# AlanLiangC/PDM-SSD

Measured on AMD Instinct MI355X. Metric: frames/sec (16384-pt clouds, bs=32), higher is better.
Workload: dtype f32; 1 GPU; configs[2]: full PDM-SSD forward (PointNet2MSG backbone + PDM neck + hybrid head: BEV heat-map head + point box head with decoded boxes), bs=32/GPU x 16384 pts, uniform KITTI-range clouds, fp32 inference, inputs resident in HBM, 4 distinct batches in rotation; launch=hipGraph, parallelism=dp1, global_batch=32

## Files before the change

include/pdmssd_hip.h:

```cpp
#ifndef PDMSSD_HIP_H
#define PDMSSD_HIP_H

#include <stddef.h>

#ifdef __cplusplus
extern "C" {
#endif

#define PDM_ABI_VERSION 1

#define PDM_E_BADARG (-1)
#define PDM_E_TOOLARGE (-2)

int pdm_abi_version(void);
const char *pdm_last_error(void);


int pdm_ball_query(void *stream, int b, int n, int m, float radius, int nsample,
                   const float *new_xyz, const float *xyz, int *idx);

int pdm_group_points(void *stream, int b, int c, int n, int npoints, int nsample,
                     const float *points, const int *idx, float *out);

int pdm_group_points_grad(void *stream, int b, int c, int n, int npoints, int nsample,
// ... 106 lines not shown
                        size_t workspace_bytes);
size_t pdm_point_head_loss_workspace_bytes(long long n_total);

int pdm_heatmap_targets(void *stream, int B, int M, int C, int H, int W, const float *gt_boxes, float x0, float y0, float vx,
                        float vy, float stride, double min_overlap, int min_radius, int max_radius, float *heatmap);
size_t pdm_heatmap_focal_loss_workspace_bytes(long long n);
int pdm_heatmap_focal_loss(void *stream, int B, int C, int H, int W, const void *logits, int logits_bf16, long long sb, long long sc,
                           long long sh, long long sw, const float *heatmap, float weight, float *dlogits, float *out,
                           void *workspace, size_t workspace_bytes);

int pdm_rows_mlp_x3(void *stream, int rows, int cin, const float *in_pm, int nlayers, const int *dims, const void *wstream,
                    size_t wstream_bytes, const float *bias, int relu_last, float *out_pm, int out_stride, int cout);
size_t pdm_rows_mlp_x3_stream_bytes(int nlayers, const int *dims);
int pdm_tune_rows_x3_wg_per_cu(int n);

int pdm_sa_mlp_fused_pre(void *stream, int b, int n, int m, int nsample, const float *xyz,
                         const float *new_xyz, const float *z_pm, int z_stride, int z_coff, const int *idx,
                         int nlayers, const int *dims, const float *wpack, const float *bias, float *out_pm,
                         int out_stride, int out_coff, int cout);
int pdm_fp_mlp_fused_pre(void *stream, int b, int n, int m, int c_skip, const float *z_pm, int z_stride,
                         const float *skip_pm, const int *idx, const float *weight, int nlayers,
                         const int *dims, const float *wpack, const float *bias, float *out_pm,
                         int out_stride, int cout);

size_t pdm_sa_pack_workspace_bytes(int b, int m);
size_t pdm_sa_pack_rows(int b, int m, int nsample);
int pdm_sa_pack(void *stream, int b, int n, int m, int nsample, const int *idx, void *workspace,
                size_t workspace_bytes, int *pack, int *meta);
int pdm_sa_pack_pair(void *stream, int b, int n, int m, const int *nsample, const int *const *idx, void *const *workspace,
                     size_t workspace_bytes, int *const *pack, int *const *meta);
int pdm_sa_mlp_packed(void *stream, int b, int n, int m, int cin, int nsample, const float *xyz,
                      const float *new_xyz, const float *feat_pm, const float *z_pm, int z_stride, int z_coff,
                      const int *pack, const int *meta, int nlayers, const int *dims, const float *wpack,
                      const float *bias, float *out_pm, int out_stride, int out_coff, int cout);

int pdm_sa_mlp_packed_pair(void *stream, int b, int n, int m, int cin, const int *nsample, const float *xyz,
                           const float *new_xyz, const float *feat_pm, const float *z_pm, int z_stride, const int *z_coff,
                           const int *const *pack, const int *const *meta, const int *nlayers, const int *const *dims,
                           const float *const *wpack, const float *const *bias, float *out_pm, int out_stride,
                           const int *out_coff, const int *cout);
int pdm_tune_sa_pair(int on);

int pdm_stack_ball_query(void *stream, int B, int M, float radius, int nsample, const float *new_xyz,
                         const int *new_xyz_batch_cnt, const float *xyz, const int *xyz_batch_cnt, int *idx);
int pdm_stack_group_points(void *stream, int B, int M, int C, int nsample, const float *features,
                           const int *features_batch_cnt, const int *idx, const int *idx_batch_cnt, float *out);
// ... 140 lines not shown
                        void *xmin, unsigned char *imax, unsigned char *imin);
int pdm_tg_dy_stats_parts(long long rows, int N);
int pdm_tg_gemm_nt_dy_bs(void *stream, long long R, int K, int N, const void *dZ, long long lddz, const void *Yp, long long ldyp,
                         const void *W, long long ldw, void *dX, long long lddx, void *dYout, long long lddy, const float *coef,
                         const float *grads, const void *Bx, long long ldbx, const float *bcoef, float *bstats);
size_t pdm_tg_wgrad_ws_bytes(long long R, int K, int N);
int pdm_tg_wgrad(void *stream, long long R, int K, int N, const void *dY, long long ldy, const void *X, long long ldx, float *dW,
                 int accumulate, void *workspace, size_t workspace_bytes, const float *x_bn_coef);
size_t pdm_tg_colsum_ws_floats(long long R, int N);
int pdm_tg_colsum(void *stream, long long R, int N, const void *Y, long long ld, float *out, float *scratch);
int pdm_tg_pack_weight(void *stream, int N, int K, const float *W, void *Wb, int ldb, void *Wt, int ldt);
int pdm_tg_pack_weight_pair(void *stream, int N, int K, const float *W, void *Wb, void *Wt, int rows_to, int cols_to);
int pdm_tg_pack_weight_many(void *stream, int njobs, const void *jobs, long long total_blocks);


int pdm_tune_fps_variant(int v);
int pdm_tune_fused_waves(int w);
int pdm_tune_fused_tiles(int t);
int pdm_tune_fused_groups(int n);
int pdm_tune_fused_wg_per_cu(int n);
int pdm_tune_fused_lds_cap(int bytes);
int pdm_tune_fused_reg(int on);
int pdm_tune_fused_gemm(int on);
int pdm_tune_fused_chain(int on);
int pdm_tune_fused_swz(int on);
int pdm_tune_bq_quad(int form);
int pdm_tune_bq_dense_ppc(int hundredths);
int pdm_tune_grid_split(int min_n);
int pdm_tune_bq_small_waves(int w);
int pdm_tune_bq_cpw(int centres);
int pdm_tune_bq_heavy(int candidates);
int pdm_tune_group_lds_floor(int bytes);
int pdm_tune_group_rows(int packed);
int pdm_tune_rows_chain_wg_per_cu(int n);
int pdm_tune_fp_head_tiles(int n);
int pdm_tune_rows_chain_dw_wg_per_cu(int n);
int pdm_tune_rows_chain_xcd(int on);
int pdm_tune_fp_chain_pad_lds(int bytes);

int pdm_copy_many(void *stream, int count, void *const *dst, const void *const *src, const size_t *bytes);
int pdm_copy_many_dyn(void *stream, int count, void *const *dst, const void *const *src, const size_t *bytes,
                      const int *const *dyn_count, const unsigned *dyn_unit);


int pdm_scatter_bev(void *stream, int B, int P, int C, int degree, const float *xyz,
                    const float *feat, const float *sh, const float *inv2s2, float ox, float oy,
// ... 37 lines not shown
```

pdm_ssd_amd/_native.py:

```python
import ctypes
import os

import torch

_HERE = os.path.dirname(os.path.abspath(__file__))
LIB_PATH = os.path.join(_HERE, "libpdmssd_hip.so")
ABI_VERSION = 1

_lib = None

_vp, _i, _f = ctypes.c_void_p, ctypes.c_int, ctypes.c_float

_SIGNATURES = {
    "pdm_ball_query": [_i, _i, _i, _f, _i, _vp, _vp, _vp],
    "pdm_ball_query_grid": [_i, _i, _i, _f, _i, _vp, _vp, _vp, _vp, ctypes.c_size_t],
    "pdm_grid_build": [_i, _i, _f, _vp, _vp, ctypes.c_size_t],
    "pdm_ball_query_grid_prebuilt": [_i, _i, _i, _f, _i, _vp, _vp, _vp, ctypes.c_size_t],
    "pdm_three_nn_grid_prebuilt": [_i, _i, _i, _vp, _vp, _vp, _vp, ctypes.c_size_t],
    "pdm_three_nn_grid": [_i, _i, _i, _vp, _vp, _vp, _vp, _vp, ctypes.c_size_t],
    "pdm_group_points": [_i, _i, _i, _i, _i, _vp, _vp, _vp],
    "pdm_group_points_grad": [_i, _i, _i, _i, _i, _vp, _vp, _vp],
    "pdm_group_points_grad_ws": [_i, _i, _i, _i, _i, _vp, _vp, _vp, _vp, ctypes.c_size_t],
    "pdm_gather_points": [_i, _i, _i, _i, _vp, _vp, _vp],
    "pdm_gather_points_grad": [_i, _i, _i, _i, _vp, _vp, _vp],
# ... 55 lines not shown
    "pdm_bn_relu_backward_stats": [_i, _i, ctypes.c_longlong, _i, ctypes.c_longlong, _vp, _vp, _vp, _vp, _vp, _i],
    "pdm_bn_relu_backward_apply": [_i, _i, ctypes.c_longlong, _i, ctypes.c_longlong, _vp, _vp, _vp, _vp, _vp, _i],
    "pdm_stack_voxel_query": [_i, _i, _i, _i, _i, _f, _i, _i, _i, _vp, _vp, _vp, _vp, _vp],
    "pdm_stack_local_neighbor_count": [_vp, _vp, _vp, _vp, _vp, _vp, _f, _i, _i, _i, _i],
    "pdm_stack_local_neighbor_fill": [_vp, _vp, _vp, _vp, _vp, _vp, ctypes.c_longlong, _f, _i, _i, _i, _i],
    "pdm_stack_query_local_neighbor_idxs": [_vp, _vp, _vp, _vp, _vp, _vp, _vp, _i, _f, _i, _i, _i, _i],
    "pdm_stack_three_nn_by_local_idxs": [_vp, _vp, _vp, _vp, _vp, _vp, ctypes.c_longlong, _i, _i],
    "pdm_stack_vector_pool_count": [_vp] * 7 + [_i, _i, _i, _f, _i, _i, _i, _i, _i],
    "pdm_stack_vector_pool": [_vp] * 10 + [_i, _i, _i, _f] + [_i] * 9,
    "pdm_stack_vector_pool_grad": [_vp, _vp, _vp, _vp, _i, _i, _i, _i, _i, _i],
    "pdm_three_nn_weights": [ctypes.c_longlong, _vp, _vp, _vp],
    "pdm_rows_mlp_fused": [_i, _i, _vp, _i, _vp, _vp, _vp, _i, _vp, _i, _i],
    "pdm_point_head_loss": [ctypes.c_longlong, _i, _i, _i, _i, _i, _vp, ctypes.c_longlong, _vp, ctypes.c_longlong, _vp, ctypes.c_longlong,
                            _vp, _vp, _vp, _vp, _vp, _f, _f, _f, _f, _f, _vp, _vp, _vp, _vp, _vp, ctypes.c_size_t],
    "pdm_heatmap_targets": [_i, _i, _i, _i, _i, _vp, _f, _f, _f, _f, _f, ctypes.c_double, _i, _i, _vp],
    "pdm_heatmap_focal_loss": [_i, _i, _i, _i, _vp, _i, ctypes.c_longlong, ctypes.c_longlong, ctypes.c_longlong, ctypes.c_longlong, _vp, _f, _vp, _vp,
                               _vp, ctypes.c_size_t],
    "pdm_rows_mlp_x3": [_i, _i, _vp, _i, _vp, _vp, ctypes.c_size_t, _vp, _i, _vp, _i, _i],
    "pdm_rows_mlp_fused_pair": [_i, _i, _vp, _i, _vp, _vp, _vp, _vp, _vp, _i, _vp, _i, _i, _vp, _i, _i],
    "pdm_fp_head_fused": [_i, _i, _i, _i, _vp, _i, _vp, _vp, _vp, _vp, _vp, _vp, _vp, _i, _i, _vp, _vp, _vp, _vp, _vp, _i, _vp, _i, _i,
                          _vp, _i, _i],
    "pdm_sa_mlp_fused_pre": [_i] * 4 + [_vp, _vp, _vp, _i, _i, _vp, _i, _vp, _vp, _vp, _vp, _i, _i, _i],
    "pdm_fp_mlp_fused_pre": [_i] * 4 + [_vp, _i, _vp, _vp, _vp, _i, _vp, _vp, _vp, _vp, _i, _i],
    "pdm_sa_pack": [_i, _i, _i, _i, _vp, _vp, ctypes.c_size_t, _vp, _vp],
    "pdm_sa_pack_pair": [_i, _i, _i, _vp, _vp, _vp, ctypes.c_size_t, _vp, _vp],
    "pdm_sa_mlp_packed_pair": [_i, _i, _i, _i, _vp, _vp, _vp, _vp, _vp, _i, _vp, _vp, _vp, _vp, _vp, _vp, _vp, _vp, _i, _vp, _vp],
    "pdm_sa_mlp_packed": [_i] * 5 + [_vp, _vp, _vp, _vp, _i, _i, _vp, _vp, _i, _vp, _vp, _vp, _vp, _i, _i, _i],
    "pdm_interp_concat_rows": [_i, _i, _i, _i, _i, _i, _vp, _i, _vp, _i, _vp, _vp, _vp],
    "pdm_interp_concat_rows_grad": [_i, _i, _i, _i, _i, _vp, _vp, _vp, _vp, _vp, ctypes.c_size_t],
    "pdm_interp_concat_rows_grad_out": [_i, _i, _i, _i, _i, _vp, _vp, _vp, _vp, _i, _vp, ctypes.c_size_t],
    "pdm_tg_gemm_nt": [ctypes.c_longlong, _i, _i, _vp, ctypes.c_longlong, _vp, ctypes.c_longlong, _vp, ctypes.c_longlong, _vp, _vp, _vp],
    "pdm_tg_gemm_nt_dy": [ctypes.c_longlong, _i, _i, _vp, ctypes.c_longlong, _vp, ctypes.c_longlong, _vp, ctypes.c_longlong, _vp, ctypes.c_longlong,
                          _vp, ctypes.c_longlong, _vp, _vp],
    "pdm_tg_gemm_nt_bs": [ctypes.c_longlong, _i, _i, _vp, ctypes.c_longlong, _vp, ctypes.c_longlong, _vp, ctypes.c_longlong, _vp,
                          ctypes.c_longlong, _vp, _vp],
    "pdm_tg_gemm_nt_dy_bs": [ctypes.c_longlong, _i, _i, _vp, ctypes.c_longlong, _vp, ctypes.c_longlong, _vp, ctypes.c_longlong, _vp,
                             ctypes.c_longlong, _vp, ctypes.c_longlong, _vp, _vp, _vp, ctypes.c_longlong, _vp, _vp],
    "pdm_bn_finalize_bwd_stats": [ctypes.c_longlong, _i, _vp, _vp, _vp, _i],
    "pdm_tg_gemm_nt_pool": [ctypes.c_longlong, _i, _i, _vp, ctypes.c_longlong, _vp, ctypes.c_longlong, _vp, ctypes.c_longlong, _vp, _vp, _vp,
                            _i, _vp, _vp, _vp, _vp],
    "pdm_bn_relu_pool_forward_kept": [_i, ctypes.c_longlong, _i, _i, _vp, _vp, _vp, _vp, _vp, _f, _f, _vp, _vp, _vp, _vp, _i, _i],
    "pdm_tg_wgrad": [ctypes.c_longlong, _i, _i, _vp, ctypes.c_longlong, _vp, ctypes.c_longlong, _vp, _i, _vp, ctypes.c_size_t, _vp],
    "pdm_bn_forward_coef": [_i, ctypes.c_longlong, _i, _vp, _vp, _vp, _f, _f, _vp, _vp, _vp, _vp],
    "pdm_bn_finalize_stats": [ctypes.c_longlong, _i, _vp, _vp, _f, _f, _vp, _vp, _vp, _vp, _i],
    "pdm_tg_colsum": [ctypes.c_longlong, _i, _vp, ctypes.c_longlong, _vp, _vp],
    "pdm_tg_pack_weight": [_i, _i, _vp, _vp, _i, _vp, _i],
    "pdm_tg_pack_weight_pair": [_i, _i, _vp, _vp, _vp, _i, _i],
    "pdm_tg_pack_weight_many": [_i, _vp, ctypes.c_longlong],
    "pdm_tune_fps_variant": None,
    "pdm_tune_fused_waves": None,
    "pdm_tune_fused_tiles": None,
    "pdm_tune_fused_groups": None,
    "pdm_tune_fused_wg_per_cu": None,
    "pdm_tune_fused_lds_cap": None,
    "pdm_tune_fused_reg": None,
    "pdm_tune_bq_quad": None,
    "pdm_tune_bq_heavy": None,
    "pdm_tune_bq_cpw": None,
    "pdm_tune_copy_variant": None,
    "pdm_tune_group_nt": None,
    "pdm_tune_group_lds_floor": None,
    "pdm_tune_copy_max_wg": None,
    "pdm_tune_bq_small_waves": None,
    "pdm_tune_bq_dense_ppc": None,
    "pdm_tune_grid_split": None,
    "pdm_tune_group_rows": None,
    "pdm_tune_fused_gemm": None,
    "pdm_tune_fused_chain": None,
    "pdm_tune_fused_pair": None,
    "pdm_tune_sa_pair": None,
    "pdm_tune_rows_x3_wg_per_cu": None,
    "pdm_tune_fp_chain_pad_lds": None,
    "pdm_tune_fp_chain_nt": None,
    "pdm_tune_fp_chain_mask": None,
    "pdm_tune_rows_chain_wg_per_cu": None,
    "pdm_tune_rows_chain_dw_wg_per_cu": None,
    "pdm_tune_fp_head_tiles": None,
    "pdm_tune_rows_chain_xcd": None,
    "pdm_tune_fused_swz": None,
    "pdm_scatter_bev": [_i, _i, _i, _i, _vp, _vp, _vp, _vp] + [_f] * 9 + [_i] * 7 + [_vp, _vp],
    "pdm_gather_bev": [_i, _i, _i, _i, _vp, _vp, _vp, _vp] + [_f] * 9 + [_i] * 6 + [_i, _f, _vp, _vp, _vp, ctypes.c_size_t],
    "pdm_bev_normalize_grad": [_i, _i, _i, _i, _i, _f, _vp, _vp, _vp, _vp, _vp],
    "pdm_bev_normalize": [_i, _i, _i, _i, _i, _i, _f, _vp, _vp],
    "pdm_scatter_bev_grad": [_i, _i, _i, _i, _vp, _vp, _vp, _vp] + [_f] * 9 + [_i] * 7 + [_vp] * 5,
    "pdm_scatter_bev_grad_normalized": [_i, _i, _i, _i, _vp, _vp, _vp, _vp] + [_f] * 9 + [_i] * 7 + [_vp, _vp, _f] + [_vp] * 4,
}
EXPORTS = ["pdm_abi_version", "pdm_last_error", "pdm_ball_query_grid_workspace_bytes",
           "pdm_three_nn_grid_workspace_bytes", "pdm_furthest_point_sampling_ws_bytes",
           "pdm_fps_max_coresident_workgroups",
           "pdm_gather_bev_workspace_bytes", "pdm_nms_workspace_bytes", "pdm_post_process_workspace_bytes", "pdm_augment_workspace_bytes", "pdm_sa_pack_workspace_bytes",
           "pdm_sa_pack_rows", "pdm_rows_mlp_x3_stream_bytes", "pdm_point_head_loss_workspace_bytes", "pdm_heatmap_focal_loss_workspace_bytes", "pdm_three_interpolate_grad_ws_bytes",
           "pdm_group_points_grad_ws_bytes", "pdm_group_concat_cl_grad_ws_bytes", "pdm_bn_parts", "pdm_bn_pool_parts",
           "pdm_tg_stats_parts", "pdm_tg_dy_stats_parts", "pdm_tg_wgrad_ws_bytes", "pdm_tg_colsum_ws_floats"] + list(_SIGNATURES)


class NativeLibraryError(RuntimeError):
    pass


def lib():
    global _lib
    if _lib is None:
        if not os.path.exists(LIB_PATH):
            raise NativeLibraryError(
                f"{LIB_PATH} not found: build it with `make -C pdm_ssd_amd/csrc` "
                "(or `python -c 'import __graft_entry__ as g; g.build()'`). "
                "pdm_ssd_amd has no CPU or PyTorch fallback for its operators.")
        l = ctypes.CDLL(LIB_PATH)
        l.pdm_abi_version.restype = _i
        l.pdm_last_error.restype = ctypes.c_char_p
        l.pdm_ball_query_grid_workspace_bytes.restype = ctypes.c_size_t
        l.pdm_ball_query_grid_workspace_bytes.argtypes = [_i, _i]
        l.pdm_furthest_point_sampling_ws_bytes.restype = ctypes.c_size_t
        l.pdm_furthest_point_sampling_ws_bytes.argtypes = [_i, _i]
        l.pdm_fps_max_coresident_workgroups.restype = _i
        l.pdm_fps_max_coresident_workgroups.argtypes = []
# ... 5 lines not shown
        l.pdm_sa_pack_workspace_bytes.restype = ctypes.c_size_t
        l.pdm_sa_pack_workspace_bytes.argtypes = [_i, _i]
        l.pdm_group_concat_cl_grad_ws_bytes.restype = ctypes.c_size_t
        l.pdm_group_concat_cl_grad_ws_bytes.argtypes = [_i, _i, _i, _i]
        l.pdm_group_points_grad_ws_bytes.restype = ctypes.c_size_t
        l.pdm_group_points_grad_ws_bytes.argtypes = [_i, _i, _i, _i]
        l.pdm_three_interpolate_grad_ws_bytes.restype = ctypes.c_size_t
        l.pdm_three_interpolate_grad_ws_bytes.argtypes = [_i, _i, _i]
        l.pdm_point_head_loss_workspace_bytes.restype = ctypes.c_size_t
        l.pdm_point_head_loss_workspace_bytes.argtypes = [ctypes.c_longlong]
        l.pdm_heatmap_focal_loss_workspace_bytes.restype = ctypes.c_size_t
        l.pdm_heatmap_focal_loss_workspace_bytes.argtypes = [ctypes.c_longlong]
        l.pdm_rows_mlp_x3_stream_bytes.restype = ctypes.c_size_t
        l.pdm_rows_mlp_x3_stream_bytes.argtypes = [_i, _vp]
        l.pdm_sa_pack_rows.restype = ctypes.c_size_t
        l.pdm_sa_pack_rows.argtypes = [_i, _i, _i]
        l.pdm_nms_workspace_bytes.argtypes = [_i]
        l.pdm_post_process_workspace_bytes.restype = ctypes.c_size_t
        l.pdm_post_process_workspace_bytes.argtypes = [_i, _i, _i]
        l.pdm_augment_workspace_bytes.restype = ctypes.c_size_t
        l.pdm_augment_workspace_bytes.argtypes = [_i, _i]
        l.pdm_bn_pool_parts.restype = _i
        l.pdm_bn_pool_parts.argtypes = [_i, ctypes.c_longlong, _i]
        l.pdm_tg_colsum_ws_floats.restype = ctypes.c_size_t
        l.pdm_tg_colsum_ws_floats.argtypes = [ctypes.c_longlong, _i]
        l.pdm_tg_stats_parts.restype = _i
        l.pdm_tg_stats_parts.argtypes = [ctypes.c_longlong, _i]
        l.pdm_tg_dy_stats_parts.restype = _i
        l.pdm_tg_dy_stats_parts.argtypes = [ctypes.c_longlong, _i]
        l.pdm_tg_wgrad_ws_bytes.restype = ctypes.c_size_t
        l.pdm_tg_wgrad_ws_bytes.argtypes = [ctypes.c_longlong, _i, _i]
        l.pdm_bn_parts.restype = _i
        l.pdm_bn_parts.argtypes = [_i, ctypes.c_longlong, _i, ctypes.c_longlong]
        if l.pdm_abi_version() != ABI_VERSION:
            raise NativeLibraryError(
                f"libpdmssd_hip.so ABI {l.pdm_abi_version()} != expected {ABI_VERSION}; rebuild it")
        for name, args in _SIGNATURES.items():
            fn = getattr(l, name)
            fn.restype = _i
            fn.argtypes = [_i] if args is None else [_vp] + args
        _lib = l
    return _lib


def call(name, stream, *args):
    l = lib()
# ... 68 lines not shown
```

pdm_ssd_amd/csrc/fused_mlp.hip:

```cpp
#include "common.h"

#include <mutex>
#include <set>

namespace pdm {

typedef float f4 __attribute__((ext_vector_type(4)));

constexpr int FM_MAXL = 4;

struct MlpDesc {
    int nlayers;
    int K[FM_MAXL + 1];
    int woff[FM_MAXL];
    int boff[FM_MAXL];
    int stage_in;
    int pool_floats;
    int relu_last;
    int lds_p, lds_q;
    int swz;
};

__device__ __forceinline__ int lds_col(int blk, int g, int pos, int swz) {
    const int q = 4 * blk + g;
// ... 1011 lines not shown
            } else {
#pragma unroll
                for (int t = 0; t < NT; ++t) v[t] = seg_max_nonneg4(v[t], L[t]);
            }
            const int c0 = 16 * mb + 4 * g;
#pragma unroll
            for (int t = 0; t < NT; ++t) {
                if (!orow[t]) continue;
                if (c0 + 4 <= a.cout) {
                    *reinterpret_cast<f4 *>(orow[t] + c0) = v[t];
                } else {
                    if (c0 < a.cout) orow[t][c0] = v[t].x;
                    if (c0 + 1 < a.cout) orow[t][c0 + 1] = v[t].y;
                    if (c0 + 2 < a.cout) orow[t][c0 + 2] = v[t].z;
                }
            }
        }
    }
#undef PDM_CHAIN
}

int rows_gemm_launch(void *stream, int rows, int cin, const float *in_pm, int k0, int c1, const float *wpack,
                     const float *bias, int relu_last, float *out_pm, int out_stride, int cout);
int rows_chain_launch(void *stream, int rows, int cin, const float *in_pm, int nlayers, const int *dims, const float *wpack,
                      const float *bias, int relu_last, float *out_pm, int out_stride, int cout, int *launched);
int rows_chain_pair_launch(void *stream, int rows, int cin, const float *in_pm, int nlayers, const int *dims, const float *wpack_a,
                           const float *bias_a, const float *wpack_b, const float *bias_b, int relu_last, float *out_a, int out_stride_a,
                           int cout_a, float *out_b, int out_stride_b, int cout_b, int *launched);
static int g_fused_chain = 1;
static int g_fused_pair = 1;
int fp_chain_launch(void *stream, int b, int n, int m, int c_skip, const float *z_pm, int z_stride, const float *skip_pm,
                    const int *idx, const float *weight, const int *dims, const float *wpack, const float *bias, float *out_pm,
                    int out_stride, int cout, int *launched);
int fp_pre_gemm_launch(void *stream, int b, int n, int m, int c_skip, const float *z_pm, int z_stride,
                       const float *skip_pm, const int *idx, const float *weight, int k1, int c2,
                       const float *wpack, const float *bias, float *out_pm, int out_stride, int cout);
static int g_fused_swz = 1;
static int g_fused_gemm = 1;
static int g_fused_reg = 1;
static int g_fused_waves = 0;
static int g_fused_tiles = 0;
static int g_fused_groups = 0;
static int g_fused_lds_cap = 152 * 1024;
static int g_fused_wg_per_cu = 32;

static int fill_desc(const char *who, MlpDesc &d, int nlayers, const int *dims, int k0_real_max, int pool_floats,
// ... 323 lines not shown

extern "C" int pdm_fp_mlp_fused_pre(void *stream, int b, int n, int m, int c_skip, const float *z_pm,
                                    int z_stride, const float *skip_pm, const int *idx, const float *weight,
                                    int nlayers, const int *dims, const float *wpack, const float *bias,
                                    float *out_pm, int out_stride, int cout) {
    return fp_fused_launch(stream, 1, 1, b, n, m, 0, c_skip, nullptr, z_pm, z_stride, skip_pm, idx, weight, nlayers, dims,
                           wpack, bias, out_pm, out_stride, cout);
}

extern "C" int pdm_rows_mlp_fused(void *stream, int rows, int cin, const float *in_pm, int nlayers,
                                  const int *dims, const float *wpack, const float *bias, int relu_last,
                                  float *out_pm, int out_stride, int cout) {
    PDM_REQUIRE(rows >= 0 && cin >= 1, PDM_E_BADARG, "rows_mlp_fused: rows=%d cin=%d", rows, cin);
    if (g_fused_chain && dims && in_pm && wpack && bias && out_pm && cout > 0 && nlayers >= 1 && nlayers <= 3 && cout <= dims[nlayers] &&
        cout <= out_stride && out_stride % 4 == 0 &&
        ((reinterpret_cast<uintptr_t>(out_pm) | reinterpret_cast<uintptr_t>(wpack) | reinterpret_cast<uintptr_t>(bias) |
          reinterpret_cast<uintptr_t>(in_pm)) & 15) == 0) {
        int launched = 0;
        const int rc = rows_chain_launch(stream, rows, cin, in_pm, nlayers, dims, wpack, bias, relu_last, out_pm, out_stride, cout,
                                         &launched);
        if (rc || launched) return rc;
    }
    if (g_fused_gemm && nlayers == 1 && dims && dims[0] % 16 == 0 && dims[1] % 16 == 0 && dims[0] >= cin && dims[0] >= 32 &&
        dims[1] >= 64 && (long long)((rows + 127) / 128) * ((dims[1] + 127) / 128) >= 256 && in_pm && wpack && bias && out_pm && cout > 0 && cout <= dims[1] && cout <= out_stride &&
        out_stride % 4 == 0 && ((reinterpret_cast<uintptr_t>(out_pm) | reinterpret_cast<uintptr_t>(wpack) |
                                 reinterpret_cast<uintptr_t>(bias)) & 15) == 0)
        return rows_gemm_launch(stream, rows, cin, in_pm, dims[0], dims[1], wpack, bias, relu_last, out_pm, out_stride, cout);
    return fp_fused_launch(stream, 2, relu_last, 1, rows, 1, 0, cin, nullptr, nullptr, 0, in_pm, nullptr, nullptr, nlayers,
                           dims, wpack, bias, out_pm, out_stride, cout);
}

extern "C" int pdm_rows_mlp_fused_pair(void *stream, int rows, int cin, const float *in_pm, int nlayers, const int *dims,
                                       const float *wpack_a, const float *bias_a, const float *wpack_b, const float *bias_b,
                                       int relu_last, float *out_a, int out_stride_a, int cout_a, float *out_b, int out_stride_b,
                                       int cout_b) {
    PDM_REQUIRE(rows >= 0 && cin >= 1, PDM_E_BADARG, "rows_mlp_fused_pair: rows=%d cin=%d", rows, cin);
    if (g_fused_chain && g_fused_pair && dims && in_pm && wpack_a && bias_a && wpack_b && bias_b && out_a && out_b && out_a != out_b &&
        nlayers == 3 && cout_a > 0 && cout_b > 0 && cout_a <= dims[nlayers] && cout_b <= dims[nlayers] && cout_a <= out_stride_a &&
        cout_b <= out_stride_b && out_stride_a % 4 == 0 && out_stride_b % 4 == 0 &&
        ((reinterpret_cast<uintptr_t>(out_a) | reinterpret_cast<uintptr_t>(out_b) | reinterpret_cast<uintptr_t>(wpack_a) |
          reinterpret_cast<uintptr_t>(wpack_b) | reinterpret_cast<uintptr_t>(bias_a) | reinterpret_cast<uintptr_t>(bias_b) |
          reinterpret_cast<uintptr_t>(in_pm)) & 15) == 0) {
        int launched = 0;
        const int rc = rows_chain_pair_launch(stream, rows, cin, in_pm, nlayers, dims, wpack_a, bias_a, wpack_b, bias_b, relu_last, out_a,
                                              out_stride_a, cout_a, out_b, out_stride_b, cout_b, &launched);
        if (rc || launched) return rc;
    }
    if (int rc = pdm_rows_mlp_fused(stream, rows, cin, in_pm, nlayers, dims, wpack_a, bias_a, relu_last, out_a, out_stride_a, cout_a)) return rc;
    return pdm_rows_mlp_fused(stream, rows, cin, in_pm, nlayers, dims, wpack_b, bias_b, relu_last, out_b, out_stride_b, cout_b);
}
// ... 1 lines not shown
```

pdm_ssd_amd/csrc/rows_gemm.hip:

```cpp
#include "common.h"

namespace pdm {

typedef float gf4 __attribute__((ext_vector_type(4)));

constexpr int RG_ROWS = 128;
constexpr int RG_BLKS = 8;
constexpr int RG_HS = 24;

struct RowsGemmArgs {
    int rows, cin, in_stride;
    int nkb, nmb;
    int cout, out_stride;
    const float *in;
    const float *wpack;
    const float *bias;
    float *out;
    float floor;
    int n, m, z_stride, c_skip;
    const float *z;
    const float *skip;
    const int *idx;
    const float *weight;
    const float *w1;
    const float *b1;
};

template <bool FP_PRE>
__global__ __launch_bounds__(512) void rows_gemm_kernel(RowsGemmArgs a) {
    __shared__ __attribute__((aligned(16))) float s_w[2][RG_BLKS * 64 * 4];
    __shared__ __attribute__((aligned(16))) float s_h[2][RG_ROWS * RG_HS];
    const int tid = threadIdx.x, lane = tid & 63;
    const int wave = __builtin_amdgcn_readfirstlane(tid >> 6);
    const int pos = lane & 15, g = lane >> 4;
    const int wp = wave >> 2, wc = wave & 3;
    int tile = blockIdx.x;
    if constexpr (FP_PRE) {
        const int tpc = a.n / RG_ROWS, nb = a.rows / a.n;
        if (gridDim.y == 1 && tpc * RG_ROWS == a.n && (nb & 7) == 0) {
            const int xcd = tile & 7, slot = tile >> 3;
            tile = ((slot / tpc) * 8 + xcd) * tpc + slot % tpc;
        }
    }
    const long long r0 = (long long)tile * RG_ROWS;
    const int mb0 = blockIdx.y * RG_BLKS;

    const int hrow = tid >> 2, part = tid & 3;
    const bool w_live = mb0 + wave < a.nmb;
    const gf4 *wsrc = reinterpret_cast<const gf4 *>(a.wpack) + ((size_t)(mb0 + wave) * a.nkb) * 64 + lane;
    const bool h_live = r0 + hrow < a.rows;
    const float *hsrc = a.in + (size_t)(r0 + hrow) * a.in_stride + 4 * part;
    const bool vec = (a.in_stride & 3) == 0 && (reinterpret_cast<uintptr_t>(a.in) & 15) == 0;

    auto load_w = [&](int kb) {
        gf4 v = {0.f, 0.f, 0.f, 0.f};
        if (w_live) v = wsrc[(size_t)kb * 64];
        return v;
    };
    const float *zb = nullptr;
    int o0 = 0, o1 = 0, o2 = 0;
    float iw0 = 0.f, iw1 = 0.f, iw2 = 0.f, sk[4] = {0.f, 0.f, 0.f, 0.f};
    if constexpr (FP_PRE) {
        if (h_live) {
            const long long row = r0 + hrow;
            const int b = (int)(row / a.n);
            zb = a.z + (size_t)b * a.m * a.z_stride + 4 * part;
            o0 = a.idx[row * 3] * a.z_stride; o1 = a.idx[row * 3 + 1] * a.z_stride; o2 = a.idx[row * 3 + 2] * a.z_stride;
            iw0 = a.weight[row * 3]; iw1 = a.weight[row * 3 + 1]; iw2 = a.weight[row * 3 + 2];
            for (int s_ = 0; s_ < a.c_skip; ++s_) sk[s_] = a.skip[row * a.c_skip + s_];
        }
    }
    struct Raw { gf4 za, zc, zd; };
    auto load_raw = [&](int kb) {
// ... 16 lines not shown
#pragma unroll
        for (int j = 0; j < 4; ++j) {
            h[j] += __fmaf_rn(iw2, zz[2][j], __fmaf_rn(iw1, zz[1][j], __fmul_rn(iw0, zz[0][j])));
            const float *wr = a.w1 + ((size_t)(c >> 4) * 64 + ((c & 15) + j)) * 4;
            for (int s_ = 0; s_ < a.c_skip; ++s_) h[j] = fmaf(wr[s_], sk[s_], h[j]);
            h[j] = fmaxf(h[j], 0.0f);
        }
        return gf4{h[0], h[1], h[2], h[3]};
    };
    auto load_h = [&](int kb) {
        gf4 v = {0.f, 0.f, 0.f, 0.f};
        if (!h_live) return v;
        const int c = 16 * kb + 4 * part;
        if (vec && c + 4 <= a.cin) return *reinterpret_cast<const gf4 *>(hsrc + 16 * kb);
        const float *p = hsrc + 16 * kb;
        if (c < a.cin) v.x = p[0];
        if (c + 1 < a.cin) v.y = p[1];
        if (c + 2 < a.cin) v.z = p[2];
        if (c + 3 < a.cin) v.w = p[3];
        return v;
    };
    auto stage = [&](int buf, gf4 w, gf4 h) {
        reinterpret_cast<gf4 *>(s_w[buf])[tid] = w;
        *reinterpret_cast<gf4 *>(&s_h[buf][hrow * RG_HS + 4 * part]) = h;
    };

    gf4 acc[2][4];
#pragma unroll
    for (int i = 0; i < 2; ++i) {
        gf4 bi = {0.f, 0.f, 0.f, 0.f};
        if (mb0 + 2 * wc + i < a.nmb) bi = *reinterpret_cast<const gf4 *>(a.bias + 16 * (mb0 + 2 * wc + i) + 4 * g);
#pragma unroll
        for (int t = 0; t < 4; ++t) acc[i][t] = bi;
    }

    gf4 gw = load_w(0), gh = {0.f, 0.f, 0.f, 0.f};
    Raw gr;
    if constexpr (FP_PRE) { gr = load_raw(0); gh = finish(gr, 0); } else gh = load_h(0);
    stage(0, gw, gh);
    __syncthreads();
    if (a.nkb > 1) {
        gw = load_w(1);
        if constexpr (FP_PRE) gr = load_raw(1); else gh = load_h(1);
    }
    for (int kb = 0; kb < a.nkb; ++kb) {
        const int cur = kb & 1;
        gf4 fa[2], fb[4];
#pragma unroll
        for (int i = 0; i < 2; ++i) fa[i] = reinterpret_cast<const gf4 *>(s_w[cur])[(2 * wc + i) * 64 + lane];
#pragma unroll
        for (int t = 0; t < 4; ++t) fb[t] = *reinterpret_cast<const gf4 *>(&s_h[cur][((4 * wp + t) * 16 + pos) * RG_HS + 4 * g]);
        if (kb + 1 < a.nkb) {
            if constexpr (FP_PRE) gh = finish(gr, kb + 1);
            stage(cur ^ 1, gw, gh);
        }
        if (kb + 2 < a.nkb) {
            gw = load_w(kb + 2);
            if constexpr (FP_PRE) gr = load_raw(kb + 2); else gh = load_h(kb + 2);
        }
#define PDM_RG_MFMA(C)                                                                                         \
    _Pragma("unroll") for (int i = 0; i < 2; ++i) _Pragma("unroll") for (int t = 0; t < 4; ++t)                 \
        acc[i][t] = __builtin_amdgcn_mfma_f32_16x16x4f32(fa[i].C, fb[t].C, acc[i][t], 0, 0, 0);
        PDM_RG_MFMA(x) PDM_RG_MFMA(y) PDM_RG_MFMA(z) PDM_RG_MFMA(w)
#undef PDM_RG_MFMA
        __syncthreads();
    }

#pragma unroll
    for (int t = 0; t < 4; ++t) {
        const long long row = r0 + (4 * wp + t) * 16 + pos;
        if (row >= a.rows) continue;
        float *orow = a.out + (size_t)row * a.out_stride;
#pragma unroll
        for (int i = 0; i < 2; ++i) {
            const int c0 = 16 * (mb0 + 2 * wc + i) + 4 * g;
            gf4 v = acc[i][t];
            v.x = __builtin_amdgcn_fmed3f(v.x, a.floor, __builtin_inff()); v.y = __builtin_amdgcn_fmed3f(v.y, a.floor, __builtin_inff());
            v.z = __builtin_amdgcn_fmed3f(v.z, a.floor, __builtin_inff()); v.w = __builtin_amdgcn_fmed3f(v.w, a.floor, __builtin_inff());
            if (c0 + 4 <= a.cout) {
                *reinterpret_cast<gf4 *>(orow + c0) = v;
            } else {
                if (c0 < a.cout) orow[c0] = v.x;
                if (c0 + 1 < a.cout) orow[c0 + 1] = v.y;
                if (c0 + 2 < a.cout) orow[c0 + 2] = v.z;
            }
        }
    }
}

int rows_gemm_launch(void *stream, int rows, int cin, const float *in_pm, int k0, int c1, const float *wpack,
                     const float *bias, int relu_last, float *out_pm, int out_stride, int cout) {
    RowsGemmArgs a;
    a.rows = rows; a.cin = cin; a.in_stride = cin;
    a.nkb = k0 >> 4; a.nmb = c1 >> 4;
    a.cout = cout; a.out_stride = out_stride;
    a.in = in_pm; a.wpack = wpack; a.bias = bias; a.out = out_pm;
    a.floor = relu_last ? 0.0f : -__builtin_inff();
    a.n = a.m = a.z_stride = a.c_skip = 0;
    a.z = a.skip = a.weight = a.w1 = a.b1 = nullptr; a.idx = nullptr;
    const dim3 grid((unsigned)((rows + RG_ROWS - 1) / RG_ROWS), (unsigned)((a.nmb + RG_BLKS - 1) / RG_BLKS));
    hipLaunchKernelGGL(rows_gemm_kernel<false>, grid, dim3(512), 0, as_stream(stream), a);
    return check_launch("rows_mlp_fused(gemm)");
}

int fp_pre_gemm_launch(void *stream, int b, int n, int m, int c_skip, const float *z_pm, int z_stride,
                       const float *skip_pm, const int *idx, const float *weight, int k1, int c2,
                       const float *wpack, const float *bias, float *out_pm, int out_stride, int cout) {
    RowsGemmArgs a;
    a.rows = b * n; a.cin = k1; a.in_stride = 0;
    a.nkb = k1 >> 4; a.nmb = c2 >> 4;
    a.cout = cout; a.out_stride = out_stride;
    a.in = nullptr; a.wpack = wpack + 16 * k1; a.bias = bias + k1; a.out = out_pm;
    a.floor = 0.0f;
    a.n = n; a.m = m; a.z_stride = z_stride; a.c_skip = c_skip;
    a.z = z_pm; a.skip = skip_pm; a.idx = idx; a.weight = weight; a.w1 = wpack; a.b1 = bias;
    const dim3 grid((unsigned)((a.rows + RG_ROWS - 1) / RG_ROWS), (unsigned)((a.nmb + RG_BLKS - 1) / RG_BLKS));
    hipLaunchKernelGGL(rows_gemm_kernel<true>, grid, dim3(512), 0, as_stream(stream), a);
    return check_launch("fp_mlp_fused_pre(gemm)");
}

}
```

pdm_ssd_amd/fused.py:

```python
import ctypes

import numpy as np
import torch
import torch.nn as nn

from . import _native

FLOP_COUNTER = None


def _count(name, positions, pk):
    if FLOP_COUNTER is not None:
        FLOP_COUNTER[name] = FLOP_COUNTER.get(name, 0.0) + float(positions) * pk.flops_per_position


def _pad16(c):
    return (c + 15) // 16 * 16


def fold_conv_bn(conv, bn):
    w = conv.weight.detach().double().reshape(conv.out_channels, conv.in_channels).cpu()
    if conv.bias is not None:
        cb = conv.bias.detach().double().cpu()
    else:
# ... 373 lines not shown
def sa_level_forward_packed(pks, xyz, new_xyz, feat_pm, z, z_coffs, packeds, nss, out_pm, out_coffs):
    B, N, _ = xyz.shape
    M = new_xyz.shape[1]
    cin = 0 if (feat_pm is None or z is not None) else feat_pm.shape[2]
    assert len(pks) == 2 and all(pk.cin == cin + 3 for pk in pks)
    if FLOP_COUNTER is not None:
        for pk, (pack, meta) in zip(pks, packeds):
            _count("pdm_sa_mlp_packed_pair", int(meta[6].item()), pk)
    I2, P2 = ctypes.c_int * 2, ctypes.c_void_p * 2
    keep = [I2(*nss), I2(*z_coffs), P2(*[p.data_ptr() for p, _ in packeds]), P2(*[m.data_ptr() for _, m in packeds]),
            I2(*[pk.nlayers for pk in pks]), P2(*[pk.dims_ptr.value for pk in pks]), P2(*[pk.wpack.data_ptr() for pk in pks]),
            P2(*[pk.bias.data_ptr() for pk in pks]), I2(*out_coffs), I2(*[pk.cout for pk in pks])]
    c = [ctypes.cast(k, ctypes.c_void_p) for k in keep]
    _native.call("pdm_sa_mlp_packed_pair", _stream(xyz), B, N, M, cin, c[0], xyz.data_ptr(), new_xyz.data_ptr(),
                 0 if cin == 0 else feat_pm.data_ptr(), 0 if z is None else z.data_ptr(), 0 if z is None else z.shape[2], c[1], c[2], c[3],
                 c[4], c[5], c[6], c[7], out_pm.data_ptr(), out_pm.shape[2], c[8], c[9])


def fp_forward_pre(pk, z, skip_pm, idx, weight, out_pm):
    B, m, _ = z.shape
    n = idx.shape[1]
    cs = 0 if skip_pm is None else skip_pm.shape[2]
    assert pk.cin == cs
    _count("pdm_fp_mlp_fused_pre", B * n, pk)
    _native.call("pdm_fp_mlp_fused_pre", _stream(z), B, n, m, cs, z.data_ptr(), z.shape[2],
                 0 if skip_pm is None else skip_pm.data_ptr(), idx.data_ptr(), weight.data_ptr(), pk.nlayers,
                 pk.dims_ptr, pk.wpack.data_ptr(), pk.bias.data_ptr(), out_pm.data_ptr(), out_pm.shape[2], pk.cout)
```

Before: 7272 frames/s.

## Add small-row-tile GEMM forms and split FP pre-MLP into interp-fused two-GEMM path

Templates the rows GEMM kernel on row-tile size (128/64/32) so under-filled launches with large K and N use smaller tiles and produce more workgroups. Adds a workspace-based FP pre path that runs the first layer as a GEMM on skip features, adds the three-NN interpolated z in the epilogue, and runs the second layer as a separate GEMM. This replaces the single fused pre kernel when grids would be small. It costs an intermediate workspace round trip through HBM and a torch allocation per call.

```diff
diff --git a/include/pdmssd_hip.h b/include/pdmssd_hip.h
--- a/include/pdmssd_hip.h
+++ b/include/pdmssd_hip.h
@@ -152,6 +152,11 @@
                          const float *skip_pm, const int *idx, const float *weight, int nlayers,
                          const int *dims, const float *wpack, const float *bias, float *out_pm,
                          int out_stride, int cout);
+size_t pdm_fp_mlp_pre_ws_floats(int b, int n, int c_skip, int nlayers, const int *dims);
+int pdm_fp_mlp_fused_pre_ws(void *stream, int b, int n, int m, int c_skip, const float *z_pm, int z_stride,
+                            const float *skip_pm, const int *idx, const float *weight, int nlayers,
+                            const int *dims, const float *wpack, const float *bias, float *out_pm,
+                            int out_stride, int cout, float *ws, size_t ws_floats);
 
 size_t pdm_sa_pack_workspace_bytes(int b, int m);
 size_t pdm_sa_pack_rows(int b, int m, int nsample);
@@ -338,6 +343,7 @@
 int pdm_tune_fused_lds_cap(int bytes);
 int pdm_tune_fused_reg(int on);
 int pdm_tune_fused_gemm(int on);
+int pdm_tune_rows_gemm_forms(int on);
 int pdm_tune_fused_chain(int on);
 int pdm_tune_fused_swz(int on);
 int pdm_tune_bq_quad(int form);
diff --git a/pdm_ssd_amd/_native.py b/pdm_ssd_amd/_native.py
--- a/pdm_ssd_amd/_native.py
+++ b/pdm_ssd_amd/_native.py
@@ -101,6 +101,7 @@
                           _vp, _i, _i],
     "pdm_sa_mlp_fused_pre": [_i] * 4 + [_vp, _vp, _vp, _i, _i, _vp, _i, _vp, _vp, _vp, _vp, _i, _i, _i],
     "pdm_fp_mlp_fused_pre": [_i] * 4 + [_vp, _i, _vp, _vp, _vp, _i, _vp, _vp, _vp, _vp, _i, _i],
+    "pdm_fp_mlp_fused_pre_ws": [_i] * 4 + [_vp, _i, _vp, _vp, _vp, _i, _vp, _vp, _vp, _vp, _i, _i, _vp, ctypes.c_size_t],
     "pdm_sa_pack": [_i, _i, _i, _i, _vp, _vp, ctypes.c_size_t, _vp, _vp],
     "pdm_sa_pack_pair": [_i, _i, _i, _vp, _vp, _vp, ctypes.c_size_t, _vp, _vp],
     "pdm_sa_mlp_packed_pair": [_i, _i, _i, _i, _vp, _vp, _vp, _vp, _vp, _i, _vp, _vp, _vp, _vp, _vp, _vp, _vp, _vp, _i, _vp, _vp],
@@ -133,6 +134,7 @@
     "pdm_tune_fused_wg_per_cu": None,
     "pdm_tune_fused_lds_cap": None,
     "pdm_tune_fused_reg": None,
+    "pdm_tune_rows_gemm_forms": None,
     "pdm_tune_bq_quad": None,
     "pdm_tune_bq_heavy": None,
     "pdm_tune_bq_cpw": None,
@@ -170,7 +172,7 @@
            "pdm_gather_bev_workspace_bytes", "pdm_nms_workspace_bytes", "pdm_post_process_workspace_bytes", "pdm_augment_workspace_bytes", "pdm_sa_pack_workspace_bytes",
            "pdm_sa_pack_rows", "pdm_rows_mlp_x3_stream_bytes", "pdm_point_head_loss_workspace_bytes", "pdm_heatmap_focal_loss_workspace_bytes", "pdm_three_interpolate_grad_ws_bytes",
            "pdm_group_points_grad_ws_bytes", "pdm_group_concat_cl_grad_ws_bytes", "pdm_bn_parts", "pdm_bn_pool_parts",
-           "pdm_tg_stats_parts", "pdm_tg_dy_stats_parts", "pdm_tg_wgrad_ws_bytes", "pdm_tg_colsum_ws_floats"] + list(_SIGNATURES)
+           "pdm_tg_stats_parts", "pdm_tg_dy_stats_parts", "pdm_tg_wgrad_ws_bytes", "pdm_tg_colsum_ws_floats", "pdm_fp_mlp_pre_ws_floats"] + list(_SIGNATURES)
 
 
 class NativeLibraryError(RuntimeError):
@@ -222,6 +224,8 @@
         l.pdm_augment_workspace_bytes.argtypes = [_i, _i]
         l.pdm_bn_pool_parts.restype = _i
         l.pdm_bn_pool_parts.argtypes = [_i, ctypes.c_longlong, _i]
+        l.pdm_fp_mlp_pre_ws_floats.restype = ctypes.c_size_t
+        l.pdm_fp_mlp_pre_ws_floats.argtypes = [_i, _i, _i, _i, _vp]
         l.pdm_tg_colsum_ws_floats.restype = ctypes.c_size_t
         l.pdm_tg_colsum_ws_floats.argtypes = [ctypes.c_longlong, _i]
         l.pdm_tg_stats_parts.restype = _i
diff --git a/pdm_ssd_amd/csrc/fused_mlp.hip b/pdm_ssd_amd/csrc/fused_mlp.hip
--- a/pdm_ssd_amd/csrc/fused_mlp.hip
+++ b/pdm_ssd_amd/csrc/fused_mlp.hip
@@ -1057,6 +1057,9 @@
 
 int rows_gemm_launch(void *stream, int rows, int cin, const float *in_pm, int k0, int c1, const float *wpack,
                      const float *bias, int relu_last, float *out_pm, int out_stride, int cout);
+bool rows_gemm_tiles_apply(int rows, int k0, int c1);
+int rows_gemm_tiles_launch(void *stream, int rows, int cin, const float *in_pm, int k0, int c1, const float *wpack,
+                           const float *bias, int relu_last, float *out_pm, int out_stride, int cout);
 int rows_chain_launch(void *stream, int rows, int cin, const float *in_pm, int nlayers, const int *dims, const float *wpack,
                       const float *bias, int relu_last, float *out_pm, int out_stride, int cout, int *launched);
 int rows_chain_pair_launch(void *stream, int rows, int cin, const float *in_pm, int nlayers, const int *dims, const float *wpack_a,
@@ -1426,10 +1429,15 @@
         if (rc || launched) return rc;
     }
     if (g_fused_gemm && nlayers == 1 && dims && dims[0] % 16 == 0 && dims[1] % 16 == 0 && dims[0] >= cin && dims[0] >= 32 &&
-        dims[1] >= 64 && (long long)((rows + 127) / 128) * ((dims[1] + 127) / 128) >= 256 && in_pm && wpack && bias && out_pm && cout > 0 && cout <= dims[1] && cout <= out_stride &&
+        dims[1] >= 64 && in_pm && wpack && bias && out_pm && cout > 0 && cout <= dims[1] && cout <= out_stride &&
         out_stride % 4 == 0 && ((reinterpret_cast<uintptr_t>(out_pm) | reinterpret_cast<uintptr_t>(wpack) |
-                                 reinterpret_cast<uintptr_t>(bias)) & 15) == 0)
-        return rows_gemm_launch(stream, rows, cin, in_pm, dims[0], dims[1], wpack, bias, relu_last, out_pm, out_stride, cout);
+                                 reinterpret_cast<uintptr_t>(bias)) & 15) == 0) {
+        if (rows_gemm_tiles_apply(rows, dims[0], dims[1]))
+            return rows_gemm_tiles_launch(stream, rows, cin, in_pm, dims[0], dims[1], wpack, bias, relu_last, out_pm, out_stride,
+                                          cout);
+        if ((long long)((rows + 127) / 128) * ((dims[1] + 127) / 128) >= 256)
+            return rows_gemm_launch(stream, rows, cin, in_pm, dims[0], dims[1], wpack, bias, relu_last, out_pm, out_stride, cout);
+    }
     return fp_fused_launch(stream, 2, relu_last, 1, rows, 1, 0, cin, nullptr, nullptr, 0, in_pm, nullptr, nullptr, nlayers,
                            dims, wpack, bias, out_pm, out_stride, cout);
 }
diff --git a/pdm_ssd_amd/csrc/rows_gemm.hip b/pdm_ssd_amd/csrc/rows_gemm.hip
--- a/pdm_ssd_amd/csrc/rows_gemm.hip
+++ b/pdm_ssd_amd/csrc/rows_gemm.hip
@@ -26,29 +26,34 @@
     const float *b1;
 };
 
-template <bool FP_PRE>
-__global__ __launch_bounds__(512) void rows_gemm_kernel(RowsGemmArgs a) {
+template <int ROWS, bool FP_PRE, bool INTERP = false>
+__device__ __forceinline__ void rows_gemm_body(const RowsGemmArgs &a) {
+    static_assert(ROWS == 128 || ROWS == 64 || ROWS == 32, "row tile");
+    static_assert(!FP_PRE || ROWS == 128, "the FP_PRE form stages with all 512 threads");
+    static_assert(!INTERP || (ROWS <= 64 && !FP_PRE), "INTERP keeps 24 RT registers of gathered z in flight");
+    constexpr int RT = ROWS / 32;
     __shared__ __attribute__((aligned(16))) float s_w[2][RG_BLKS * 64 * 4];
-    __shared__ __attribute__((aligned(16))) float s_h[2][RG_ROWS * RG_HS];
+    __shared__ __attribute__((aligned(16))) float s_h[2][ROWS * RG_HS];
     const int tid = threadIdx.x, lane = tid & 63;
     const int wave = __builtin_amdgcn_readfirstlane(tid >> 6);
     const int pos = lane & 15, g = lane >> 4;
     const int wp = wave >> 2, wc = wave & 3;
     int tile = blockIdx.x;
     if constexpr (FP_PRE) {
-        const int tpc = a.n / RG_ROWS, nb = a.rows / a.n;
-        if (gridDim.y == 1 && tpc * RG_ROWS == a.n && (nb & 7) == 0) {
+        const int tpc = a.n / ROWS, nb = a.rows / a.n;
+        if (gridDim.y == 1 && tpc * ROWS == a.n && (nb & 7) == 0) {
             const int xcd = tile & 7, slot = tile >> 3;
             tile = ((slot / tpc) * 8 + xcd) * tpc + slot % tpc;
         }
     }
-    const long long r0 = (long long)tile * RG_ROWS;
+    const long long r0 = (long long)tile * ROWS;
     const int mb0 = blockIdx.y * RG_BLKS;
 
     const int hrow = tid >> 2, part = tid & 3;
     const bool w_live = mb0 + wave < a.nmb;
     const gf4 *wsrc = reinterpret_cast<const gf4 *>(a.wpack) + ((size_t)(mb0 + wave) * a.nkb) * 64 + lane;
-    const bool h_live = r0 + hrow < a.rows;
+    const bool h_role = ROWS == 128 || hrow < ROWS;
+    const bool h_live = h_role && r0 + hrow < a.rows;
     const float *hsrc = a.in + (size_t)(r0 + hrow) * a.in_stride + 4 * part;
     const bool vec = (a.in_stride & 3) == 0 && (reinterpret_cast<uintptr_t>(a.in) & 15) == 0;
 
@@ -111,16 +116,42 @@
     };
     auto stage = [&](int buf, gf4 w, gf4 h) {
         reinterpret_cast<gf4 *>(s_w[buf])[tid] = w;
-        *reinterpret_cast<gf4 *>(&s_h[buf][hrow * RG_HS + 4 * part]) = h;
-    };
-
-    gf4 acc[2][4];
+        if (h_role) *reinterpret_cast<gf4 *>(&s_h[buf][hrow * RG_HS + 4 * part]) = h;
+    };
+
+    gf4 acc[2][RT];
 #pragma unroll
     for (int i = 0; i < 2; ++i) {
         gf4 bi = {0.f, 0.f, 0.f, 0.f};
         if (mb0 + 2 * wc + i < a.nmb) bi = *reinterpret_cast<const gf4 *>(a.bias + 16 * (mb0 + 2 * wc + i) + 4 * g);
 #pragma unroll
-        for (int t = 0; t < 4; ++t) acc[i][t] = bi;
+        for (int t = 0; t < RT; ++t) acc[i][t] = bi;
+    }
+
+    constexpr int ZT = INTERP ? RT : 1;
+    gf4 zp[ZT][2][3];
+    float zw[ZT][3];
+    if constexpr (INTERP) {
+#pragma unroll
+        for (int t = 0; t < RT; ++t) {
+            const long long row = r0 + (RT * wp + t) * 16 + pos;
+            const bool live = row < a.rows;
+            const long long rr = live ? row : 0;
+            const float *zb = a.z + (size_t)(rr / a.n) * a.m * a.z_stride;
+            const float *zr[3] = {zb + (size_t)a.idx[rr * 3] * a.z_stride, zb + (size_t)a.idx[rr * 3 + 1] * a.z_stride,
+                                  zb + (size_t)a.idx[rr * 3 + 2] * a.z_stride};
+#pragma unroll
+            for (int k = 0; k < 3; ++k) zw[t][k] = a.weight[rr * 3 + k];
+#pragma unroll
+            for (int i = 0; i < 2; ++i) {
+                const int mb = mb0 + 2 * wc + i;
+#pragma unroll
+                for (int k = 0; k < 3; ++k) {
+                    zp[t][i][k] = gf4{0.f, 0.f, 0.f, 0.f};
+                    if (live && mb < a.nmb) zp[t][i][k] = *reinterpret_cast<const gf4 *>(zr[k] + 16 * mb + 4 * g);
+                }
+            }
+        }
     }
 
     gf4 gw = load_w(0), gh = {0.f, 0.f, 0.f, 0.f};
@@ -134,11 +165,11 @@
     }
     for (int kb = 0; kb < a.nkb; ++kb) {
         const int cur = kb & 1;
-        gf4 fa[2], fb[4];
+        gf4 fa[2], fb[RT];
 #pragma unroll
         for (int i = 0; i < 2; ++i) fa[i] = reinterpret_cast<const gf4 *>(s_w[cur])[(2 * wc + i) * 64 + lane];
 #pragma unroll
-        for (int t = 0; t < 4; ++t) fb[t] = *reinterpret_cast<const gf4 *>(&s_h[cur][((4 * wp + t) * 16 + pos) * RG_HS + 4 * g]);
+        for (int t = 0; t < RT; ++t) fb[t] = *reinterpret_cast<const gf4 *>(&s_h[cur][((RT * wp + t) * 16 + pos) * RG_HS + 4 * g]);
         if (kb + 1 < a.nkb) {
             if constexpr (FP_PRE) gh = finish(gr, kb + 1);
             stage(cur ^ 1, gw, gh);
@@ -148,7 +179,7 @@
             if constexpr (FP_PRE) gr = load_raw(kb + 2); else gh = load_h(kb + 2);
         }
 #define PDM_RG_MFMA(C)                                                                                         \
-    _Pragma("unroll") for (int i = 0; i < 2; ++i) _Pragma("unroll") for (int t = 0; t < 4; ++t)                 \
+    _Pragma("unroll") for (int i = 0; i < 2; ++i) _Pragma("unroll") for (int t = 0; t < RT; ++t)                \
         acc[i][t] = __builtin_amdgcn_mfma_f32_16x16x4f32(fa[i].C, fb[t].C, acc[i][t], 0, 0, 0);
         PDM_RG_MFMA(x) PDM_RG_MFMA(y) PDM_RG_MFMA(z) PDM_RG_MFMA(w)
 #undef PDM_RG_MFMA
@@ -156,14 +187,23 @@
     }
 
 #pragma unroll
-    for (int t = 0; t < 4; ++t) {
-        const long long row = r0 + (4 * wp + t) * 16 + pos;
+    for (int t = 0; t < RT; ++t) {
+        const long long row = r0 + (RT * wp + t) * 16 + pos;
         if (row >= a.rows) continue;
         float *orow = a.out + (size_t)row * a.out_stride;
 #pragma unroll
         for (int i = 0; i < 2; ++i) {
             const int c0 = 16 * (mb0 + 2 * wc + i) + 4 * g;
             gf4 v = acc[i][t];
+            if constexpr (INTERP) {
+                if (mb0 + 2 * wc + i >= a.nmb) continue;
+                const gf4 p0 = zp[t][i][0], p1 = zp[t][i][1], p2 = zp[t][i][2];
+                const float w0 = zw[t][0], w1 = zw[t][1], w2 = zw[t][2];
+                v.x += __fmaf_rn(w2, p2.x, __fmaf_rn(w1, p1.x, __fmul_rn(w0, p0.x)));
+                v.y += __fmaf_rn(w2, p2.y, __fmaf_rn(w1, p1.y, __fmul_rn(w0, p0.y)));
+                v.z += __fmaf_rn(w2, p2.z, __fmaf_rn(w1, p1.z, __fmul_rn(w0, p0.z)));
+                v.w += __fmaf_rn(w2, p2.w, __fmaf_rn(w1, p1.w, __fmul_rn(w0, p0.w)));
+            }
             v.x = __builtin_amdgcn_fmed3f(v.x, a.floor, __builtin_inff()); v.y = __builtin_amdgcn_fmed3f(v.y, a.floor, __builtin_inff());
             v.z = __builtin_amdgcn_fmed3f(v.z, a.floor, __builtin_inff()); v.w = __builtin_amdgcn_fmed3f(v.w, a.floor, __builtin_inff());
             if (c0 + 4 <= a.cout) {
@@ -176,6 +216,15 @@
         }
     }
 }
+
+template <bool FP_PRE>
+__global__ __launch_bounds__(512) void rows_gemm_kernel(RowsGemmArgs a) { rows_gemm_body<RG_ROWS, FP_PRE>(a); }
+template <int ROWS>
+__global__ __launch_bounds__(512) void rows_gemm_tile_kernel(RowsGemmArgs a) { rows_gemm_body<ROWS, false>(a); }
+template <int ROWS>
+__global__ __launch_bounds__(512) void rows_gemm_interp_kernel(RowsGemmArgs a) { rows_gemm_body<ROWS, false, true>(a); }
+
+static int g_rows_gemm_tiles = 1;
 
 int rows_gemm_launch(void *stream, int rows, int cin, const float *in_pm, int k0, int c1, const float *wpack,
                      const float *bias, int relu_last, float *out_pm, int out_stride, int cout) {
@@ -191,6 +240,88 @@
     hipLaunchKernelGGL(rows_gemm_kernel<false>, grid, dim3(512), 0, as_stream(stream), a);
     return check_launch("rows_mlp_fused(gemm)");
 }
+
+static int rows_gemm_small_tile(int rows, int c1) {
+    const long long cblk = (c1 / 16 + RG_BLKS - 1) / RG_BLKS;
+    if (!g_rows_gemm_tiles || rows <= 0 || (long long)(rows + 127) / 128 * cblk >= 512) return 0;
+    return (long long)(rows + 63) / 64 * cblk >= 512 ? 64 : 32;
+}
+bool rows_gemm_tiles_apply(int rows, int k0, int c1) { return k0 >= 256 && c1 >= 256 && rows_gemm_small_tile(rows, c1) != 0; }
+int rows_gemm_tiles_launch(void *stream, int rows, int cin, const float *in_pm, int k0, int c1, const float *wpack,
+                           const float *bias, int relu_last, float *out_pm, int out_stride, int cout) {
+    RowsGemmArgs a;
+    a.rows = rows; a.cin = cin; a.in_stride = cin;
+    a.nkb = k0 >> 4; a.nmb = c1 >> 4;
+    a.cout = cout; a.out_stride = out_stride;
+    a.in = in_pm; a.wpack = wpack; a.bias = bias; a.out = out_pm;
+    a.floor = relu_last ? 0.0f : -__builtin_inff();
+    a.n = a.m = a.z_stride = a.c_skip = 0;
+    a.z = a.skip = a.weight = a.w1 = a.b1 = nullptr; a.idx = nullptr;
+    const int rt = rows_gemm_small_tile(rows, c1);
+    const dim3 grid((unsigned)((rows + rt - 1) / rt), (unsigned)((a.nmb + RG_BLKS - 1) / RG_BLKS));
+    if (rt == 64) hipLaunchKernelGGL(rows_gemm_tile_kernel<64>, grid, dim3(512), 0, as_stream(stream), a);
+    else hipLaunchKernelGGL(rows_gemm_tile_kernel<32>, grid, dim3(512), 0, as_stream(stream), a);
+    return check_launch("rows_mlp_fused(gemm tiles)");
+}
+
+static long long fp_two_gemm_ws_floats(int b, int n, int c_skip, int nlayers, const int *dims) {
+    if (!g_rows_gemm_tiles || b <= 0 || n <= 0 || nlayers != 2 || !dims || c_skip < 16) return 0;
+    for (int l = 0; l <= 2; ++l)
+        if (dims[l] <= 0 || dims[l] % 16) return 0;
+    if (dims[0] < c_skip || dims[1] < 384 || dims[2] < 256) return 0;
+    const long long rows = (long long)b * n;
+    if (rows >= (1ll << 31) || rows * dims[1] >= (1ll << 40)) return 0;
+    if ((rows + RG_ROWS - 1) / RG_ROWS * ((dims[2] / 16 + RG_BLKS - 1) / RG_BLKS) < 512) return 0;
+    return rows * dims[1];
+}
+
+}
+
+using namespace pdm;
+
+extern "C" size_t pdm_fp_mlp_pre_ws_floats(int b, int n, int c_skip, int nlayers, const int *dims) {
+    return (size_t)fp_two_gemm_ws_floats(b, n, c_skip, nlayers, dims);
+}
+
+extern "C" int pdm_fp_mlp_fused_pre(void *stream, int b, int n, int m, int c_skip, const float *z_pm, int z_stride,
+                                    const float *skip_pm, const int *idx, const float *weight, int nlayers, const int *dims,
+                                    const float *wpack, const float *bias, float *out_pm, int out_stride, int cout);
+extern "C" int pdm_fp_mlp_fused_pre_ws(void *stream, int b, int n, int m, int c_skip, const float *z_pm, int z_stride,
+                                       const float *skip_pm, const int *idx, const float *weight, int nlayers,
+                                       const int *dims, const float *wpack, const float *bias, float *out_pm,
+                                       int out_stride, int cout, float *ws, size_t ws_floats) {
+    const long long need = fp_two_gemm_ws_floats(b, n, c_skip, nlayers, dims);
+    if (need == 0 || !ws || ws_floats < (size_t)need)
+        return pdm_fp_mlp_fused_pre(stream, b, n, m, c_skip, z_pm, z_stride, skip_pm, idx, weight, nlayers, dims, wpack, bias,
+                                    out_pm, out_stride, cout);
+    PDM_REQUIRE(m >= 1 && z_pm && skip_pm && idx && weight && wpack && bias && out_pm, PDM_E_BADARG,
+                "fp_mlp_fused_pre_ws: null pointer or m=%d", m);
+    const int k1 = dims[1], c2 = dims[2];
+    PDM_REQUIRE(z_stride % 4 == 0 && z_stride >= k1 && (long long)m * z_stride < (1ll << 31), PDM_E_BADARG,
+                "fp_mlp_fused_pre_ws: z rows need %d floats, stride %d (multiple of 4)", k1, z_stride);
+    PDM_REQUIRE(cout > 0 && cout <= c2 && cout <= out_stride && out_stride % 4 == 0, PDM_E_BADARG,
+                "fp_mlp_fused_pre_ws: cout=%d stride=%d", cout, out_stride);
+    PDM_REQUIRE(((reinterpret_cast<uintptr_t>(z_pm) | reinterpret_cast<uintptr_t>(out_pm) | reinterpret_cast<uintptr_t>(ws) |
+                  reinterpret_cast<uintptr_t>(wpack) | reinterpret_cast<uintptr_t>(bias)) & 15) == 0,
+                PDM_E_BADARG, "fp_mlp_fused_pre_ws: buffers must be 16-byte aligned");
+    const int rows = b * n;
+    RowsGemmArgs a;
+    a.rows = rows; a.cin = c_skip; a.in_stride = c_skip;
+    a.nkb = dims[0] >> 4; a.nmb = k1 >> 4;
+    a.cout = k1; a.out_stride = k1;
+    a.in = skip_pm; a.wpack = wpack; a.bias = bias; a.out = ws;
+    a.floor = 0.0f;
+    a.n = n; a.m = m; a.z_stride = z_stride; a.c_skip = 0;
+    a.z = z_pm; a.idx = idx; a.weight = weight; a.skip = nullptr; a.w1 = a.b1 = nullptr;
+    const int rt = (long long)(rows + 63) / 64 * ((a.nmb + RG_BLKS - 1) / RG_BLKS) >= 512 ? 64 : 32;
+    const dim3 grid((unsigned)((rows + rt - 1) / rt), (unsigned)((a.nmb + RG_BLKS - 1) / RG_BLKS));
+    if (rt == 64) hipLaunchKernelGGL(rows_gemm_interp_kernel<64>, grid, dim3(512), 0, as_stream(stream), a);
+    else hipLaunchKernelGGL(rows_gemm_interp_kernel<32>, grid, dim3(512), 0, as_stream(stream), a);
+    if (int rc = check_launch("fp_mlp_fused_pre_ws(layer 1)")) return rc;
+    return rows_gemm_launch(stream, rows, k1, ws, k1, c2, wpack + (size_t)dims[0] * k1, bias + k1, 1, out_pm, out_stride, cout);
+}
+
+namespace pdm {
 
 int fp_pre_gemm_launch(void *stream, int b, int n, int m, int c_skip, const float *z_pm, int z_stride,
                        const float *skip_pm, const int *idx, const float *weight, int k1, int c2,
@@ -209,3 +340,5 @@
 }
 
 }
+
+extern "C" int pdm_tune_rows_gemm_forms(int on) { const int old = g_rows_gemm_tiles; g_rows_gemm_tiles = on != 0; return old; }
diff --git a/pdm_ssd_amd/fused.py b/pdm_ssd_amd/fused.py
--- a/pdm_ssd_amd/fused.py
+++ b/pdm_ssd_amd/fused.py
@@ -419,6 +419,15 @@
     n = idx.shape[1]
     cs = 0 if skip_pm is None else skip_pm.shape[2]
     assert pk.cin == cs
+    ws_floats = _native.lib().pdm_fp_mlp_pre_ws_floats(B, n, cs, pk.nlayers, pk.dims_ptr)
+    if ws_floats:
+        ws = torch.empty(ws_floats, dtype=torch.float32, device=z.device)
+        _count("pdm_fp_mlp_fused_pre_ws", B * n, pk)
+        _native.call("pdm_fp_mlp_fused_pre_ws", _stream(z), B, n, m, cs, z.data_ptr(), z.shape[2],
+                     0 if skip_pm is None else skip_pm.data_ptr(), idx.data_ptr(), weight.data_ptr(), pk.nlayers,
+                     pk.dims_ptr, pk.wpack.data_ptr(), pk.bias.data_ptr(), out_pm.data_ptr(), out_pm.shape[2], pk.cout,
+                     ws.data_ptr(), ws_floats)
+        return
     _count("pdm_fp_mlp_fused_pre", B * n, pk)
     _native.call("pdm_fp_mlp_fused_pre", _stream(z), B, n, m, cs, z.data_ptr(), z.shape[2],
                  0 if skip_pm is None else skip_pm.data_ptr(), idx.data_ptr(), weight.data_ptr(), pk.nlayers,
```

After: 7450 frames/s, median of 6. 1.02x the previous value.
